# tlkvstepan/PracticalDeepStereo_NIPS2018

Measured on AMD Instinct MI355X. Metric: stereo pairs/sec, 960x540 D=192, Matching+Regularization+SubpixelMap hot path, higher is better.
Workload: dtype f32; 1 GPU; configs[1]: 960x540 pair padded to 576x960, D=192 (48 matching planes, 96 cost planes), batch 1, eval mode, random-init weights seed 0; parallelism=single GPU, launch=eager, whole pairs round-robin over 3 HIP streams

## Files before the change

practicaldeepstereo_nips2018_amd/csrc/conv2d_t8.hip:

```cpp
#include <atomic>
#include <type_traits>

#include "common.hpp"

namespace pds {

namespace {

constexpr int C2_THREADS = 256;
constexpr int C2_CIN = 64, C2_COUT = 8, C2_KC = 4, C2_CHUNKS = C2_CIN / C2_KC;
constexpr int C2_TY = 16, C2_NB = 2, C2_TX = 16 * C2_NB, C2_RP = C2_TY / 8;
constexpr int C2_YT = C2_TY + 2, C2_XT = C2_TX + 2, C2_RS = 36;
constexpr int C2_PART = C2_YT * C2_RS * 8;
constexpr int C2_BUF = 2 * C2_PART;
constexpr int C2_AFRAGS = C2_CHUNKS * 3 * 2;
constexpr int C2_ABYTES = C2_AFRAGS * 64 * 8;
constexpr int C2_NPOS = C2_YT * C2_XT;
constexpr int C2_POS = (C2_NPOS + C2_THREADS - 1) / C2_THREADS;
static_assert(C2_RS >= C2_XT, "LDS row");
typedef float f32x4 __attribute__((ext_vector_type(4)));
typedef _Float16 f16x4 __attribute__((ext_vector_type(4)));

struct C2Args {
    Src a, b;
    const float* __restrict__ w;
    const float* __restrict__ bias;
    float* __restrict__ out;
    int N, D, H, W;
    int lrelu;
    int tiles_x, tiles_y, tiles;
};

__device__ __forceinline__ void c2_split(const float (&v)[4], f16x4& hi, f16x4& lo) {
    pds_u32x2 h, l;
    split_quad_f16(v, h, l);
    hi = __builtin_bit_cast(f16x4, h);
    lo = __builtin_bit_cast(f16x4, l);
}

struct C2Scales {
    float ws, as, unscale;
};
__device__ __forceinline__ float c2_uniform(float v) {
    return __builtin_bit_cast(float, __builtin_amdgcn_readfirstlane(__builtin_bit_cast(int, v)));
}
__device__ __forceinline__ C2Scales c2_scales(const C2Args& A, bool two, float* red) {
    float m[3] = {0.f, 0.f, 0.f};
    for (int i = threadIdx.x; i < C2_COUT * C2_CIN * 9; i += blockDim.x) m[0] = fmaxf(m[0], fabsf(A.w[i]));
    for (int i = threadIdx.x; i < A.a.bound_n; i += blockDim.x) {
        const float v = fabsf(A.a.bound[i]);
        m[1] = fmaxf(m[1], v == v ? v : __builtin_inff());
    }
    if (two)
        for (int i = threadIdx.x; i < A.b.bound_n; i += blockDim.x) {
            const float v = fabsf(A.b.bound[i]);
            m[2] = fmaxf(m[2], v == v ? v : __builtin_inff());
        }
    const int wave = threadIdx.x >> 6, waves = (blockDim.x + 63) >> 6;
#pragma unroll
    for (int k = 0; k < 3; ++k) {
        m[k] = wave_max(m[k]);
        if ((threadIdx.x & 63) == 0) red[wave * 3 + k] = m[k];
    }
    __syncthreads();
    float r[3] = {0.f, 0.f, 0.f};
    for (int w = 0; w < waves; ++w)
#pragma unroll
        for (int k = 0; k < 3; ++k) r[k] = fmaxf(r[k], red[w * 3 + k]);
    __syncthreads();
    C2Scales S;
    S.ws = c2_uniform(pow2_scale(r[0], kHalfTarget));
    S.as = c2_uniform(pow2_scale(r[1] + r[2], kHalfTarget));
    S.unscale = c2_uniform((1.f / S.ws) * (1.f / S.as));
    return S;
}

}

template <bool TWO, bool NA, bool NB2>
__global__ __launch_bounds__(C2_THREADS, 2) void conv2d_t8_kernel(const C2Args A) {
    extern __shared__ __attribute__((aligned(16))) unsigned char lds[];
    unsigned char* abuf = lds;
    unsigned char* ibuf = lds + C2_ABYTES;

    const int tid = threadIdx.x;
    const int lane = tid & 63;
    const int wave = __builtin_amdgcn_readfirstlane(tid >> 6);
    const int n16 = lane & 15, q = lane >> 4;
    const size_t plane = (size_t)A.H * A.W;
    const size_t cstride = (size_t)A.D * plane;
    const int cbytes = (int)(cstride * sizeof(float));
    const __amdgpu_buffer_rsrc_t ra = __builtin_amdgcn_make_buffer_rsrc(
        const_cast<float*>(A.a.p), 0, (int)((size_t)A.N * C2_CIN * cstride * sizeof(float)), 0x00020000);
    const __amdgpu_buffer_rsrc_t rb = __builtin_amdgcn_make_buffer_rsrc(
        const_cast<float*>(TWO ? A.b.p : A.a.p), 0, (int)((size_t)A.N * C2_CIN * cstride * sizeof(float)), 0x00020000);
    const __amdgpu_buffer_rsrc_t ro = __builtin_amdgcn_make_buffer_rsrc(
        A.out, 0, (int)((size_t)A.N * C2_COUT * cstride * sizeof(float)), 0x00020000);

    const C2Scales SC = c2_scales(A, TWO, reinterpret_cast<float*>(ibuf));
    for (int e = tid; e < C2_CHUNKS * 3 * 64; e += C2_THREADS) {
        const int l = e & 63, f = e >> 6;
        const int m = l & 15, oc = m >> 1, py = m & 1, yi = l >> 4, dy = yi - py;
        const int chunk = f / 3, dx = f % 3;
        float wv[4];
#pragma unroll
        for (int i = 0; i < 4; ++i)
            wv[i] = (dy >= 0 && dy <= 2)
                        ? A.w[((size_t)oc * C2_CIN + chunk * C2_KC + i) * 9 + dy * 3 + dx] * SC.ws
                        : 0.f;
        f16x4 hi, lo;
        c2_split(wv, hi, lo);
        *reinterpret_cast<f16x4*>(abuf + ((size_t)(f * 2 + 0) * 64 + l) * 8) = hi;
        *reinterpret_cast<f16x4*>(abuf + ((size_t)(f * 2 + 1) * 64 + l) * 8) = lo;
    }

    const int xcd = blockIdx.x & 7, slot = blockIdx.x >> 3, per_xcd = gridDim.x >> 3;
    const int t_end = (int)(((long long)(xcd + 1) * A.tiles) >> 3);
    const int t_first = (int)(((long long)xcd * A.tiles) >> 3) + slot;
    const int my_tiles = t_first < t_end ? (t_end - t_first + per_xcd - 1) / per_xcd : 0;
    const int total_chunks = my_tiles * C2_CHUNKS;

    int lo_off[C2_POS];
#pragma unroll
    for (int k = 0; k < C2_POS; ++k) {
        const int p = min(tid + C2_THREADS * k, C2_NPOS - 1);
        lo_off[k] = ((p / C2_XT) * C2_RS + p % C2_XT) * 8;
    }

    struct TilePos {
        int nb, d, y0, x0;
    };
    auto tile_pos = [&](int local) {
        const int t = t_first + min(local, my_tiles - 1) * per_xcd;
        TilePos p;
        p.x0 = (t % A.tiles_x) * C2_TX;
        int r = t / A.tiles_x;
        p.y0 = (r % A.tiles_y) * C2_TY;
        r /= A.tiles_y;
        p.d = r % A.D;
        p.nb = r / A.D;
        return p;
    };

    unsigned goff[C2_POS], goff_n[C2_POS];
    float inside[C2_POS], inside_n[C2_POS];
    int sbase = 0, sbase_n = 0;
    int gidx = 0, gidx_n = 0, gch = 0, gch_n = 0;
    const int stride_a = (NA && A.a.per_plane) ? A.D : 1, stride_b = (TWO && NB2 && A.b.per_plane) ? A.D : 1;
    auto prepare = [&](int local, unsigned* off, float* in, int& sb, int& gi, int& gc) {
        const TilePos P = tile_pos(local);
#pragma unroll
        for (int k = 0; k < C2_POS; ++k) {
            const int p = min(tid + C2_THREADS * k, C2_NPOS - 1);
            const int y = P.y0 + p / C2_XT - 1, x = P.x0 + p % C2_XT - 1;
            const bool ok = (unsigned)y < (unsigned)A.H && (unsigned)x < (unsigned)A.W;
            in[k] = ok ? 1.f : 0.f;
            off[k] = ok ? (unsigned)((size_t)y * A.W + x) * 4u : ~0u;
        }
        sb = (int)(((size_t)P.nb * C2_CIN * A.D + P.d) * plane * sizeof(float));
        gi = (NA && A.a.per_plane) ? P.nb * C2_CIN * A.D + P.d : P.nb * C2_CIN;
        gc = (TWO && NB2 && A.b.per_plane) ? P.nb * C2_CIN * A.D + P.d : P.nb * C2_CIN;
    };

    constexpr int DEPTH = 4;
    float va[DEPTH][C2_POS][C2_KC], vb[DEPTH][C2_POS][C2_KC];
    float vs[DEPTH][C2_KC], vh[DEPTH][C2_KC], vs2[DEPTH][C2_KC], vh2[DEPTH][C2_KC];
    float inside_regs[DEPTH][C2_POS];
    auto fetch = [&](int g, auto set_c) {
        constexpr int SET = decltype(set_c)::value;
        const int c0 = (g % C2_CHUNKS) * C2_KC;
        const int soff = __builtin_amdgcn_readfirstlane(sbase + c0 * cbytes);
#pragma unroll
        for (int k = 0; k < C2_POS; ++k) {
#pragma unroll
            for (int ch = 0; ch < C2_KC; ++ch) {
                va[SET][k][ch] =
                    __builtin_bit_cast(float, __builtin_amdgcn_raw_buffer_load_b32(ra, goff[k], soff + ch * cbytes, 0));
                if (TWO)
                    vb[SET][k][ch] = __builtin_bit_cast(
                        float, __builtin_amdgcn_raw_buffer_load_b32(rb, goff[k], soff + ch * cbytes, 0));
            }
            inside_regs[SET][k] = inside[k];
        }
#pragma unroll
        for (int ch = 0; ch < C2_KC; ++ch) {
            if (NA) {
                const int gi = __builtin_amdgcn_readfirstlane(gidx + (c0 + ch) * stride_a);
                vs[SET][ch] = A.a.scale[gi];
                vh[SET][ch] = A.a.shift[gi];
            }
            if (TWO && NB2) {
                const int gi = __builtin_amdgcn_readfirstlane(gch + (c0 + ch) * stride_b);
                vs2[SET][ch] = A.b.scale[gi];
                vh2[SET][ch] = A.b.shift[gi];
            }
        }
    };
    auto stash = [&](unsigned char* buf, auto set_c) {
        constexpr int SET = decltype(set_c)::value;
        float cs[C2_KC], cs2[C2_KC], chs[C2_KC];
#pragma unroll
        for (int ch = 0; ch < C2_KC; ++ch) {
            cs[ch] = NA ? vs[SET][ch] * SC.as : SC.as;
            cs2[ch] = (TWO && NB2) ? vs2[SET][ch] * SC.as : SC.as;
            chs[ch] = ((NA ? vh[SET][ch] : 0.f) + ((TWO && NB2) ? vh2[SET][ch] : 0.f)) * SC.as;
        }
#pragma unroll
        for (int k = 0; k < C2_POS; ++k) {
            float v[4];
#pragma unroll
            for (int ch = 0; ch < C2_KC; ++ch) {
                float t = cs[ch] * va[SET][k][ch];
                if (TWO) t = fmaf(cs2[ch], vb[SET][k][ch], t);
                if (NA || (TWO && NB2)) t = fmaf(chs[ch], inside_regs[SET][k], t);
                v[ch] = t;
            }
            f16x4 hi, lo;
            c2_split(v, hi, lo);
            *reinterpret_cast<f16x4*>(buf + lo_off[k]) = hi;
            *reinterpret_cast<f16x4*>(buf + C2_PART + lo_off[k]) = lo;
        }
    };

    const float bscale = SC.ws * SC.as;
    const float bias0 = (A.bias ? A.bias[2 * q] : 0.f) * bscale, bias1 = (A.bias ? A.bias[2 * q + 1] : 0.f) * bscale;
    const int b_base = ((2 * C2_RP * wave + q) * C2_RS + n16) * 8;
    const unsigned out_lane = (unsigned)((size_t)(2 * q) * cstride + n16) * 4u;
    const unsigned out_c1 = (unsigned)cstride * 4u;

    using S0 = std::integral_constant<int, 0>;
    using S1 = std::integral_constant<int, 1>;
    using S2 = std::integral_constant<int, 2>;
    using S3 = std::integral_constant<int, 3>;
    int fetched_tile = -1;
    auto fetch_chunk = [&](int g, auto set_c) {
        const int gf = min(g, total_chunks - 1);
        if (gf / C2_CHUNKS != fetched_tile) {
            fetched_tile = gf / C2_CHUNKS;
            prepare(fetched_tile, goff, inside, sbase, gidx, gch);
        }
        fetch(gf, set_c);
    };
    if (total_chunks > 0) {
        fetch_chunk(0, S0());
        stash(ibuf, S0());
        fetch_chunk(1, S1());
        fetch_chunk(2, S2());
        fetch_chunk(3, S3());
    }
    __syncthreads();

    f32x4 acc[C2_RP][C2_NB];
    TilePos Pcur = tile_pos(0);
    auto step = [&](int g, auto set_stash, auto set_fetch) {
        const int c = g % C2_CHUNKS;
        if (c == 0) {
            Pcur = tile_pos(g / C2_CHUNKS);
#pragma unroll
            for (int p = 0; p < C2_RP; ++p)
#pragma unroll
                for (int j = 0; j < C2_NB; ++j) acc[p][j] = f32x4{bias0, bias0, bias1, bias1};
        }
        const int gf = min(g + DEPTH, total_chunks - 1);
        const bool new_tile = gf / C2_CHUNKS != fetched_tile;
        if (new_tile) prepare(gf / C2_CHUNKS, goff_n, inside_n, sbase_n, gidx_n, gch_n);
        fetched_tile = gf / C2_CHUNKS;

        const unsigned char* buf = ibuf + (g & 1) * C2_BUF + b_base;
        stash(ibuf + ((g + 1) & 1) * C2_BUF, set_stash);
#pragma unroll
        for (int k = 0; k < C2_POS; ++k) {
            inside[k] = new_tile ? inside_n[k] : inside[k];
            goff[k] = new_tile ? goff_n[k] : goff[k];
        }
        sbase = new_tile ? sbase_n : sbase;
        gidx = new_tile ? gidx_n : gidx;
        gch = new_tile ? gch_n : gch;
        fetch(gf, set_fetch);
        const unsigned char* af = abuf + ((size_t)c * 3 * 2 * 64 + lane) * 8;
#pragma unroll
        for (int dx = 0; dx < 3; ++dx) {
            const f16x4 a_hi = *reinterpret_cast<const f16x4*>(af + (dx * 2 + 0) * 512);
            const f16x4 a_lo = *reinterpret_cast<const f16x4*>(af + (dx * 2 + 1) * 512);
#pragma unroll
            for (int p = 0; p < C2_RP; ++p)
#pragma unroll
                for (int j = 0; j < C2_NB; ++j) {
                    const unsigned char* bp = buf + ((2 * p) * C2_RS + 16 * j + dx) * 8;
                    const f16x4 b_hi = *reinterpret_cast<const f16x4*>(bp);
                    const f16x4 b_lo = *reinterpret_cast<const f16x4*>(bp + C2_PART);
                    acc[p][j] = __builtin_amdgcn_mfma_f32_16x16x16f16(a_hi, b_lo, acc[p][j], 0, 0, 0);
                    acc[p][j] = __builtin_amdgcn_mfma_f32_16x16x16f16(a_lo, b_hi, acc[p][j], 0, 0, 0);
                    acc[p][j] = __builtin_amdgcn_mfma_f32_16x16x16f16(a_hi, b_hi, acc[p][j], 0, 0, 0);
                }
        }
#pragma unroll
        for (int i = 0; i < 3 * C2_RP * C2_NB * 3; ++i) {
            __builtin_amdgcn_sched_group_barrier(0x008, 1, 0);
            __builtin_amdgcn_sched_group_barrier(0x100, 1, 0);
            __builtin_amdgcn_sched_group_barrier(0x002, 4, 0);
            __builtin_amdgcn_sched_group_barrier(0x200, 1, 0);
            __builtin_amdgcn_sched_group_barrier(0x020, 1, 0);
        }
        if (c == C2_CHUNKS - 1) {
            const int out_base = (int)((size_t)Pcur.nb * C2_COUT * cstride * sizeof(float));
#pragma unroll
            for (int p = 0; p < C2_RP; ++p)
#pragma unroll
                for (int r = 0; r < 4; ++r) {
                    const int h = r >> 1, y = Pcur.y0 + 2 * (C2_RP * wave + p) + (r & 1);
                    const int row_bytes = __builtin_amdgcn_readfirstlane(
                        out_base + (int)(((size_t)Pcur.d * A.H + min(y, A.H - 1)) * A.W + Pcur.x0) * (int)sizeof(float));
#pragma unroll
                    for (int j = 0; j < C2_NB; ++j) {
                        float t = acc[p][j][r] * SC.unscale;
                        if (A.lrelu) t = fmaxf(t, t * kLeakySlope);
                        const bool ok = y < A.H && Pcur.x0 + 16 * j + n16 < A.W;
                        __builtin_amdgcn_raw_buffer_store_b32(__builtin_bit_cast(int, t), ro,
                                                              ok ? out_lane + (h ? out_c1 : 0u) + 64u * j : ~0u, row_bytes, 0);
                    }
                }
        }
        __syncthreads();
    };
    for (int g = 0; g < total_chunks; g += 4) {
        step(g, S1(), S0());
        step(g + 1, S2(), S1());
        step(g + 2, S3(), S2());
        step(g + 3, S0(), S3());
    }
}

constexpr int C2W_THREADS = 512;
constexpr int C2W_MAXW = 352;
typedef unsigned u32x4 __attribute__((ext_vector_type(4)));

template <bool TWO, int NBH, int C2W_TY, int C2W_ITEMS>
__global__ __launch_bounds__(C2W_THREADS, 2) void conv2d_t8w_kernel(const C2Args A) {
    constexpr int C2W_YT = C2W_TY + 2;
    extern __shared__ __attribute__((aligned(16))) unsigned char lds[];
    unsigned char* abuf = lds;
    unsigned char* ibuf = lds + C2_ABYTES;
    const int RSW = A.W + 4, QW = A.W >> 2;
    const int part_bytes = C2W_YT * RSW * 8, buf_bytes = 2 * part_bytes;

    const int tid = threadIdx.x;
    const int lane = tid & 63;
    const int wave = __builtin_amdgcn_readfirstlane(tid >> 6);
    const int pair = wave & 3, half = wave >> 2;
    const int n16 = lane & 15, q = lane >> 4;
    const size_t plane = (size_t)A.H * A.W;
    const size_t cstride = (size_t)A.D * plane;
    const int cbytes = (int)(cstride * sizeof(float));
    const __amdgpu_buffer_rsrc_t ra = __builtin_amdgcn_make_buffer_rsrc(
        const_cast<float*>(A.a.p), 0, (int)((size_t)A.N * C2_CIN * cstride * sizeof(float)), 0x00020000);
    const __amdgpu_buffer_rsrc_t rb = __builtin_amdgcn_make_buffer_rsrc(
        const_cast<float*>(TWO ? A.b.p : A.a.p), 0, (int)((size_t)A.N * C2_CIN * cstride * sizeof(float)), 0x00020000);
    const __amdgpu_buffer_rsrc_t ro = __builtin_amdgcn_make_buffer_rsrc(
        A.out, 0, (int)((size_t)A.N * C2_COUT * cstride * sizeof(float)), 0x00020000);

    const C2Scales SC = c2_scales(A, TWO, reinterpret_cast<float*>(ibuf));
    for (int e = tid; e < C2_CHUNKS * 3 * 64; e += C2W_THREADS) {
        const int l = e & 63, f = e >> 6;
        const int m = l & 15, oc = m >> 1, py = m & 1, yi = l >> 4, dy = yi - py;
        const int chunk = f / 3, dx = f % 3;
        float wv[4];
#pragma unroll
        for (int i = 0; i < 4; ++i)
            wv[i] = (dy >= 0 && dy <= 2)
                        ? A.w[((size_t)oc * C2_CIN + chunk * C2_KC + i) * 9 + dy * 3 + dx] * SC.ws
                        : 0.f;
        f16x4 hi, lo;
        c2_split(wv, hi, lo);
        *reinterpret_cast<f16x4*>(abuf + ((size_t)(f * 2 + 0) * 64 + l) * 8) = hi;
        *reinterpret_cast<f16x4*>(abuf + ((size_t)(f * 2 + 1) * 64 + l) * 8) = lo;
    }
    for (int e = tid; e < 2 * 2 * C2W_YT * 2; e += C2W_THREADS) {
        const int side = e & 1, row = e >> 1;
        *reinterpret_cast<unsigned long long*>(ibuf + ((size_t)row * RSW + (side ? A.W + 2 : 1)) * 8) = 0ull;
    }

    const int xcd = blockIdx.x & 7, slot = blockIdx.x >> 3, per_xcd = gridDim.x >> 3;
    const int t_end = (int)(((long long)(xcd + 1) * A.tiles) >> 3);
    const int t_first = (int)(((long long)xcd * A.tiles) >> 3) + slot;
    const int my_tiles = t_first < t_end ? (t_end - t_first + per_xcd - 1) / per_xcd : 0;
    const int total_chunks = my_tiles * C2_CHUNKS;

    int item_row[C2W_ITEMS], item_col[C2W_ITEMS], lo_off[C2W_ITEMS], lo_step[C2W_ITEMS];
    bool item_ok[C2W_ITEMS];
#pragma unroll
    for (int k = 0; k < C2W_ITEMS; ++k) {
        item_ok[k] = tid + C2W_THREADS * k < C2W_YT * QW;
        const int it = min(tid + C2W_THREADS * k, C2W_YT * QW - 1);
        item_row[k] = it / QW;
        item_col[k] = 4 * (it % QW);
        lo_off[k] = item_ok[k] ? (item_row[k] * RSW + 2 + item_col[k]) * 8 : 0;
        lo_step[k] = item_ok[k] ? 16 : 0;
    }

    struct TilePos {
        int nb, d, y0;
    };
    auto tile_pos = [&](int local) {
        const int t = t_first + min(local, my_tiles - 1) * per_xcd;
        TilePos p;
        p.y0 = (t % A.tiles_y) * C2W_TY;
        const int r = t / A.tiles_y;
        p.d = r % A.D;
        p.nb = r / A.D;
        return p;
    };

    unsigned goff[C2W_ITEMS], goff_n[C2W_ITEMS];
    float inside[C2W_ITEMS], inside_n[C2W_ITEMS];
    int sbase = 0, sbase_n = 0;
    int gidx = 0, gidx_n = 0;
    const int stride_a = A.a.per_plane ? A.D : 1;
    auto prepare = [&](int local, unsigned* off, float* in, int& sb, int& gi) {
        const TilePos P = tile_pos(local);
#pragma unroll
        for (int k = 0; k < C2W_ITEMS; ++k) {
            const int y = P.y0 + item_row[k] - 1;
            const bool ok = (unsigned)y < (unsigned)A.H && item_ok[k];
            in[k] = ok ? 1.f : 0.f;
            off[k] = ok ? (unsigned)((size_t)y * A.W + item_col[k]) * 4u : ~0u;
        }
        sb = (int)(((size_t)P.nb * C2_CIN * A.D + P.d) * plane * sizeof(float));
        gi = A.a.per_plane ? P.nb * C2_CIN * A.D + P.d : P.nb * C2_CIN;
    };

    f32x4 va[2][C2W_ITEMS][C2_KC], vb[2][C2W_ITEMS][C2_KC];
    float vs[2][C2_KC], vh[2][C2_KC];
    float inside_regs[2][C2W_ITEMS];
    auto fetch = [&](int g, auto set_c) {
        constexpr int SET = decltype(set_c)::value;
        const int c0 = (g % C2_CHUNKS) * C2_KC;
        const int soff = __builtin_amdgcn_readfirstlane(sbase + c0 * cbytes);
#pragma unroll
        for (int k = 0; k < C2W_ITEMS; ++k) {
#pragma unroll
            for (int ch = 0; ch < C2_KC; ++ch) {
                va[SET][k][ch] = __builtin_bit_cast(
                    f32x4, __builtin_amdgcn_raw_buffer_load_b128(ra, goff[k], soff + ch * cbytes, 0));
                if (TWO)
                    vb[SET][k][ch] = __builtin_bit_cast(
                        f32x4, __builtin_amdgcn_raw_buffer_load_b128(rb, goff[k], soff + ch * cbytes, 0));
            }
            inside_regs[SET][k] = inside[k];
        }
#pragma unroll
        for (int ch = 0; ch < C2_KC; ++ch) {
            const int gi = __builtin_amdgcn_readfirstlane(gidx + (c0 + ch) * stride_a);
            vs[SET][ch] = A.a.scale[gi];
            vh[SET][ch] = A.a.shift[gi];
        }
    };
    typedef _Float16 f16x8 __attribute__((ext_vector_type(8)));
    auto stash = [&](unsigned char* buf, auto set_c) {
        constexpr int SET = decltype(set_c)::value;
        float cs[C2_KC], chs[C2_KC];
#pragma unroll
        for (int ch = 0; ch < C2_KC; ++ch) {
            cs[ch] = vs[SET][ch] * SC.as;
            chs[ch] = vh[SET][ch] * SC.as;
        }
#pragma unroll
        for (int k = 0; k < C2W_ITEMS; ++k)
#pragma unroll
            for (int pp = 0; pp < 2; ++pp) {
                f16x8 hi2, lo2;
#pragma unroll
                for (int e = 0; e < 2; ++e) {
                    const int px = 2 * pp + e;
                    float v[4];
#pragma unroll
                    for (int ch = 0; ch < C2_KC; ++ch) {
                        float t = cs[ch] * va[SET][k][ch][px];
                        if (TWO) t = fmaf(SC.as, vb[SET][k][ch][px], t);
                        v[ch] = fmaf(chs[ch], inside_regs[SET][k], t);
                    }
                    f16x4 hi, lo;
                    c2_split(v, hi, lo);
#pragma unroll
                    for (int i = 0; i < 4; ++i) {
                        hi2[4 * e + i] = hi[i];
                        lo2[4 * e + i] = lo[i];
                    }
                }
                *reinterpret_cast<f16x8*>(buf + lo_off[k] + pp * lo_step[k]) = hi2;
                *reinterpret_cast<f16x8*>(buf + part_bytes + lo_off[k] + pp * lo_step[k]) = lo2;
            }
    };

    const float bscale = SC.ws * SC.as;
    const float bias0 = (A.bias ? A.bias[2 * q] : 0.f) * bscale, bias1 = (A.bias ? A.bias[2 * q + 1] : 0.f) * bscale;
    const int b_base = ((2 * pair + q) * RSW + 16 * half * NBH + n16 + 1) * 8;
    const unsigned out_lane = (unsigned)((size_t)(2 * q) * cstride + 16 * half * NBH + n16) * 4u;
    const unsigned out_c1 = (unsigned)cstride * 4u;

    using S0 = std::integral_constant<int, 0>;
    using S1 = std::integral_constant<int, 1>;
    int fetched_tile = -1;
    auto fetch_chunk = [&](int g, auto set_c) {
        const int gf = min(g, total_chunks - 1);
        if (gf / C2_CHUNKS != fetched_tile) {
            fetched_tile = gf / C2_CHUNKS;
            prepare(fetched_tile, goff, inside, sbase, gidx);
        }
        fetch(gf, set_c);
    };
    __syncthreads();
    if (total_chunks > 0) {
        fetch_chunk(0, S0());
        stash(ibuf, S0());
        fetch_chunk(1, S1());
        fetch_chunk(2, S0());
    }
    __syncthreads();

    f32x4 acc[NBH];
    TilePos Pcur = tile_pos(0);
#ifdef PDS_C2W_TIMING
    long long tmw[5] = {0, 0, 0, 0, 0};
#endif
    auto step = [&](int g, auto set_c) {
        const int c = g % C2_CHUNKS;
        if (c == 0) {
            Pcur = tile_pos(g / C2_CHUNKS);
#pragma unroll
            for (int j = 0; j < NBH; ++j) acc[j] = f32x4{bias0, bias0, bias1, bias1};
        }
        const int gf = min(g + 3, total_chunks - 1);
        const bool new_tile = gf / C2_CHUNKS != fetched_tile;
        if (new_tile) prepare(gf / C2_CHUNKS, goff_n, inside_n, sbase_n, gidx_n);
        fetched_tile = gf / C2_CHUNKS;

        const unsigned char* buf = ibuf + (g & 1) * buf_bytes + b_base;
#ifdef PDS_C2W_TIMING
        const long long tt0 = __builtin_readcyclecounter();
#endif
        stash(ibuf + ((g + 1) & 1) * buf_bytes, set_c);
#ifdef PDS_C2W_TIMING
        asm volatile("s_waitcnt lgkmcnt(0)" ::: "memory");
        const long long tt1 = __builtin_readcyclecounter();
#endif
#pragma unroll
        for (int k = 0; k < C2W_ITEMS; ++k) {
            inside[k] = new_tile ? inside_n[k] : inside[k];
            goff[k] = new_tile ? goff_n[k] : goff[k];
        }
        sbase = new_tile ? sbase_n : sbase;
        gidx = new_tile ? gidx_n : gidx;
        fetch(gf, set_c);
#ifdef PDS_C2W_TIMING
        const long long tt2 = __builtin_readcyclecounter();
#endif
        const unsigned char* af = abuf + ((size_t)c * 3 * 2 * 64 + lane) * 8;
#pragma unroll
        for (int dx = 0; dx < 3; ++dx) {
            const f16x4 a_hi = *reinterpret_cast<const f16x4*>(af + (dx * 2 + 0) * 512);
            const f16x4 a_lo = *reinterpret_cast<const f16x4*>(af + (dx * 2 + 1) * 512);
#pragma unroll
            for (int j = 0; j < NBH; ++j) {
                const unsigned char* bp = buf + (16 * j + dx) * 8;
                const f16x4 b_hi = *reinterpret_cast<const f16x4*>(bp);
                const f16x4 b_lo = *reinterpret_cast<const f16x4*>(bp + part_bytes);
                acc[j] = __builtin_amdgcn_mfma_f32_16x16x16f16(a_hi, b_lo, acc[j], 0, 0, 0);
                acc[j] = __builtin_amdgcn_mfma_f32_16x16x16f16(a_lo, b_hi, acc[j], 0, 0, 0);
                acc[j] = __builtin_amdgcn_mfma_f32_16x16x16f16(a_hi, b_hi, acc[j], 0, 0, 0);
            }
        }
#ifndef PDS_C2W_TIMING
#pragma unroll
        for (int i = 0; i < 3 * NBH * 3; ++i) {
            __builtin_amdgcn_sched_group_barrier(0x008, 1, 0);
            __builtin_amdgcn_sched_group_barrier(0x100, 1, 0);
            __builtin_amdgcn_sched_group_barrier(0x002, 4, 0);
            __builtin_amdgcn_sched_group_barrier(0x200, 1, 0);
            __builtin_amdgcn_sched_group_barrier(0x020, 1, 0);
        }
#else
        const long long tt3 = __builtin_readcyclecounter();
        tmw[0] += tt1 - tt0; tmw[1] += tt2 - tt1; tmw[2] += tt3 - tt2;
#endif
        if (c == C2_CHUNKS - 1) {
            const int out_base = (int)((size_t)Pcur.nb * C2_COUT * cstride * sizeof(float));
#pragma unroll
            for (int r = 0; r < 4; ++r) {
                const int h = r >> 1, y = Pcur.y0 + 2 * pair + (r & 1);
                const int row_bytes = __builtin_amdgcn_readfirstlane(
                    out_base + (int)(((size_t)Pcur.d * A.H + min(y, A.H - 1)) * A.W) * (int)sizeof(float));
#pragma unroll
                for (int j = 0; j < NBH; ++j) {
                    float t = acc[j][r] * SC.unscale;
                    if (A.lrelu) t = fmaxf(t, t * kLeakySlope);
                    const bool ok = 2 * pair < C2W_TY && y < A.H && 16 * (half * NBH + j) + n16 < A.W;
                    __builtin_amdgcn_raw_buffer_store_b32(__builtin_bit_cast(int, t), ro,
                                                          ok ? out_lane + (h ? out_c1 : 0u) + 64u * j : ~0u, row_bytes, 0);
                }
            }
        }
#ifdef PDS_C2W_TIMING
        const long long tt4 = __builtin_readcyclecounter();
#endif
        __syncthreads();
#ifdef PDS_C2W_TIMING
        tmw[3] += __builtin_readcyclecounter() - tt4;
        tmw[4] += 1;
#endif
    };
#ifdef PDS_C2W_TIMING
    const long long t_all = __builtin_readcyclecounter();
#endif
    for (int g = 0; g < total_chunks; g += 2) {
        step(g, S1());
        step(g + 1, S0());
    }
#ifdef PDS_C2W_TIMING
    if (lane == 0 && (blockIdx.x % 61) == 0 && (wave == 0 || wave == 5))
        printf("[t8w] wg %d wave %d: total %lld | stash(+wait) %lld fetch-issue %lld mfma %lld barrier %lld over %lld chunks (%d tiles)\n",
               (int)blockIdx.x, wave, (long long)__builtin_readcyclecounter() - t_all, tmw[0], tmw[1], tmw[2], tmw[3], tmw[4], my_tiles);
#endif
}

namespace {

bool c2t8_enabled() {
    static const bool on = []() {
        const char* e = debug_switch("PDS_CONV2D_T8");
        return !(e && e[0] == '0');
    }();
    return on;
}

template <bool TWO, bool NA, bool NB2>
int launch_c2t8(const C2Args& A, hipStream_t s) {
    constexpr size_t lds_bytes = (size_t)C2_ABYTES + 2 * C2_BUF;
    static std::atomic<unsigned> attr_done{0};
    if (DeviceOnce once{attr_done}) {
        (void)hipFuncSetAttribute(reinterpret_cast<const void*>(&conv2d_t8_kernel<TWO, NA, NB2>),
                                  hipFuncAttributeMaxDynamicSharedMemorySize, (int)(160 * 1024));
    }
    int wgs = 512;
    if (wgs > A.tiles) wgs = (A.tiles + 7) / 8 * 8;
    hipLaunchKernelGGL((conv2d_t8_kernel<TWO, NA, NB2>), dim3(wgs), dim3(C2_THREADS), lds_bytes, s, A);
    return check_launch("conv2d_t8");
}

}

bool c2t8_wide(const ConvLayer& L) {
    static const bool on = []() {
        const char* e = debug_switch("PDS_CONV2D_T8W");
        return !(e && e[0] == '0');
    }();
    if (!on) return false;
    if (!L.a.scale || (L.b.p && L.b.scale)) return false;
    return (L.in.w & 3) == 0 && L.in.w >= 64 && L.in.w <= C2W_MAXW && L.in.h >= 8;
}

template <bool TWO, int NBH, int TY, int ITEMS>
int launch_c2t8w(C2Args& A, hipStream_t s) {
    A.tiles_x = 1;
    A.tiles_y = (A.H + TY - 1) / TY;
    A.tiles = A.N * A.D * A.tiles_y;
    const size_t lds_bytes = (size_t)C2_ABYTES + 2 * 2 * (size_t)(TY + 2) * (A.W + 4) * 8 + 2 * (size_t)(A.W + 4) * 8 + 256;
    static std::atomic<unsigned> attr_done{0};
    static int cus[32] = {0};
    int dev = 0;
    (void)hipGetDevice(&dev);
    if (DeviceOnce once{attr_done}) {
        (void)hipFuncSetAttribute(reinterpret_cast<const void*>(&conv2d_t8w_kernel<TWO, NBH, TY, ITEMS>),
                                  hipFuncAttributeMaxDynamicSharedMemorySize, (int)(160 * 1024));
        int n = 0;
        (void)hipDeviceGetAttribute(&n, hipDeviceAttributeMultiprocessorCount, dev);
        cus[dev & 31] = n > 0 ? n : 256;
    }
    int wgs = cus[dev & 31] / 8 * 8;
    if (wgs > A.tiles) wgs = (A.tiles + 7) / 8 * 8;
    const int probe = probe_before("conv2d_t8w", s);
    hipLaunchKernelGGL((conv2d_t8w_kernel<TWO, NBH, TY, ITEMS>), dim3(wgs), dim3(C2W_THREADS), lds_bytes, s, A);
    probe_after(probe, A.tiles, s);
    return check_launch("conv2d_t8w");
}

int c2t8w_rows(int w) {
    static const int forced = []() {
        const char* e = debug_switch("PDS_CONV2D_T8W_ROWS");
        return e ? atoi(e) : 0;
    }();
    if (forced == 8 || forced == 6) return forced;
    return 8 * (w >> 2) <= C2W_THREADS ? 6 : 8;
}

bool conv2d_t8_supported(const ConvLayer& L) {
    if (!c2t8_enabled()) return false;
    if (L.kd != 1 || L.stride != 1 || L.in.c != C2_CIN || L.out_g.c != C2_COUT) return false;
    if (L.l0A || L.side_out || L.plane_weight_sets > 0) return false;
    if (!L.a.bounded) return false;
    if (L.b.p && !L.b.bounded) return false;
    if (L.b.p && L.b.bcast_d) return false;
    if ((size_t)L.in.n * C2_CIN * L.in.d * L.in.h * L.in.w >= ((size_t)1 << 29)) return false;
    const long tiles = (long)L.in.n * L.in.d * ((L.in.h + C2_TY - 1) / C2_TY) * ((L.in.w + C2_TX - 1) / C2_TX);
    return tiles < (1L << 30);
}

int launch_conv2d_t8(const ConvLayer& L, hipStream_t s) {
    C2Args A;
    A.a = L.a;
    A.b = L.b;
    A.w = L.weight;
    A.bias = L.bias;
    A.out = L.out;
    A.N = L.in.n;
    A.D = L.in.d;
    A.H = L.in.h;
    A.W = L.in.w;
    A.lrelu = L.lrelu;
    A.tiles_x = (A.W + C2_TX - 1) / C2_TX;
    A.tiles_y = (A.H + C2_TY - 1) / C2_TY;
    A.tiles = A.N * A.D * A.tiles_y * A.tiles_x;
    if (!A.a.bound || A.a.bound_n <= 0 || (L.b.p && (!A.b.bound || A.b.bound_n <= 0)))
        return set_error(-1, "conv2d_t8: a source without a range bound");
    if (c2t8_wide(L)) {
        const int blocks = (A.W + 15) / 16, nbh = (blocks + 1) / 2;
        const int rows = c2t8w_rows(A.W), items = ((rows + 2) * (A.W >> 2) + C2W_THREADS - 1) / C2W_THREADS;
        if (nbh <= 8 && rows == 6 && items == 1)
            return L.b.p ? launch_c2t8w<true, 8, 6, 1>(A, s) : launch_c2t8w<false, 8, 6, 1>(A, s);
        if (nbh <= 8) return L.b.p ? launch_c2t8w<true, 8, 8, 2>(A, s) : launch_c2t8w<false, 8, 8, 2>(A, s);
        return L.b.p ? launch_c2t8w<true, 11, 8, 2>(A, s) : launch_c2t8w<false, 11, 8, 2>(A, s);
    }
    const bool na = L.a.scale != nullptr, nb2 = L.b.p && L.b.scale;
    if (L.b.p) {
        if (na) return nb2 ? launch_c2t8<true, true, true>(A, s) : launch_c2t8<true, true, false>(A, s);
        return nb2 ? launch_c2t8<true, false, true>(A, s) : launch_c2t8<true, false, false>(A, s);
    }
    return na ? launch_c2t8<false, true, false>(A, s) : launch_c2t8<false, false, false>(A, s);
}

}
```

Baseline: 431.6 pairs/s.

## Add warp-specialized wide conv2d kernel with dedicated staging and MFMA waves

Adds a new wide-tile conv2d kernel in which four waves only issue MFMAs while another 256 threads act as staging waves. The staging waves prefetch inputs through a deep register ring of buffer loads, apply normalization, and write split f16 hi/lo data into double-buffered LDS. Each MFMA wave covers a full row width (NB=16 or 22 blocks). The kernel is on by default and selected ahead of the existing t8w path. It aims to overlap global fetch with MFMA compute without the old kernel's interleaved stash and fetch phases, at the cost of higher register pressure and half the waves doing no math.

```diff
diff --git a/practicaldeepstereo_nips2018_amd/csrc/conv2d_t8.hip b/practicaldeepstereo_nips2018_amd/csrc/conv2d_t8.hip
--- a/practicaldeepstereo_nips2018_amd/csrc/conv2d_t8.hip
+++ b/practicaldeepstereo_nips2018_amd/csrc/conv2d_t8.hip
@@ -621,6 +621,294 @@
         printf("[t8w] wg %d wave %d: total %lld | stash(+wait) %lld fetch-issue %lld mfma %lld barrier %lld over %lld chunks (%d tiles)\n",
                (int)blockIdx.x, wave, (long long)__builtin_readcyclecounter() - t_all, tmw[0], tmw[1], tmw[2], tmw[3], tmw[4], my_tiles);
 #endif
+}
+
+namespace {
+
+constexpr int C2R_STAGERS = 256;
+typedef const __attribute__((address_space(4))) float c2r_cfloat;
+
+__device__ __forceinline__ void c2r_barrier() { asm volatile("s_waitcnt lgkmcnt(0)\n\ts_barrier" ::: "memory"); }
+
+struct C2rList {
+    int t_first, per_xcd, my_tiles, total_chunks;
+};
+__device__ __forceinline__ C2rList c2r_list(const C2Args& A) {
+    C2rList L;
+    const int xcd = blockIdx.x & 7, slot = blockIdx.x >> 3;
+    L.per_xcd = gridDim.x >> 3;
+    const int t_end = (int)(((long long)(xcd + 1) * A.tiles) >> 3);
+    L.t_first = (int)(((long long)xcd * A.tiles) >> 3) + slot;
+    L.my_tiles = L.t_first < t_end ? (t_end - L.t_first + L.per_xcd - 1) / L.per_xcd : 0;
+    L.total_chunks = L.my_tiles * C2_CHUNKS;
+    return L;
+}
+template <int TY>
+__device__ __forceinline__ void c2r_tile(const C2Args& A, const C2rList& L, int local, int& nb, int& d, int& y0) {
+    const int t = L.t_first + local * L.per_xcd;
+    y0 = (t % A.tiles_y) * TY;
+    const int r = t / A.tiles_y;
+    d = r % A.D;
+    nb = r / A.D;
+}
+
+template <int NB, int TY>
+__device__ __forceinline__ void c2r_mfma_waves(const C2Args& A, const C2Scales& SC, const C2rList& L,
+                                               const unsigned char* lds, int wave, int lane) {
+    const unsigned char* abuf = lds;
+    const unsigned char* ibuf = lds + C2_ABYTES;
+    const int RSW = A.W + 4;
+    const int part_bytes = (TY + 2) * RSW * 8, buf_bytes = 2 * part_bytes;
+    const int n16 = lane & 15, q = lane >> 4;
+    const size_t cstride = (size_t)A.D * A.H * A.W;
+    const __amdgpu_buffer_rsrc_t ro = __builtin_amdgcn_make_buffer_rsrc(
+        A.out, 0, (int)((size_t)A.N * C2_COUT * cstride * sizeof(float)), 0x00020000);
+    const float bscale = SC.ws * SC.as;
+    const float bias0 = (A.bias ? A.bias[2 * q] : 0.f) * bscale, bias1 = (A.bias ? A.bias[2 * q + 1] : 0.f) * bscale;
+    const int b_base = ((2 * wave + q) * RSW + n16 + 1) * 8;
+    const unsigned out_lane = (unsigned)((size_t)(2 * q) * cstride + n16) * 4u;
+    const unsigned out_c1 = (unsigned)cstride * 4u;
+    const bool active = 2 * wave < TY;
+    __builtin_amdgcn_s_setprio(3);
+
+    c2r_barrier();
+    for (int t = 0; t < L.my_tiles; ++t) {
+        f32x4 acc[NB];
+#pragma unroll
+        for (int j = 0; j < NB; ++j) acc[j] = f32x4{bias0, bias0, bias1, bias1};
+        for (int c = 0; c < C2_CHUNKS; ++c) {
+            if (active) {
+                const unsigned char* buf = ibuf + (c & 1) * buf_bytes + b_base;
+                const unsigned char* af = abuf + ((size_t)c * 3 * 2 * 64 + lane) * 8;
+#pragma unroll
+                for (int dx = 0; dx < 3; ++dx) {
+                    const f16x4 a_hi = *reinterpret_cast<const f16x4*>(af + (dx * 2 + 0) * 512);
+                    const f16x4 a_lo = *reinterpret_cast<const f16x4*>(af + (dx * 2 + 1) * 512);
+#pragma unroll
+                    for (int j = 0; j < NB; ++j) {
+                        const unsigned char* bp = buf + (16 * j + dx) * 8;
+                        const f16x4 b_hi = *reinterpret_cast<const f16x4*>(bp);
+                        const f16x4 b_lo = *reinterpret_cast<const f16x4*>(bp + part_bytes);
+                        acc[j] = __builtin_amdgcn_mfma_f32_16x16x16f16(a_hi, b_lo, acc[j], 0, 0, 0);
+                        acc[j] = __builtin_amdgcn_mfma_f32_16x16x16f16(a_lo, b_hi, acc[j], 0, 0, 0);
+                        acc[j] = __builtin_amdgcn_mfma_f32_16x16x16f16(a_hi, b_hi, acc[j], 0, 0, 0);
+                    }
+                }
+            }
+            c2r_barrier();
+        }
+        if (active) {
+            int nb, d, y0;
+            c2r_tile<TY>(A, L, t, nb, d, y0);
+            const int out_base = (int)((size_t)nb * C2_COUT * cstride * sizeof(float));
+#pragma unroll
+            for (int r = 0; r < 4; ++r) {
+                const int h = r >> 1, y = y0 + 2 * wave + (r & 1);
+                const int row_bytes = __builtin_amdgcn_readfirstlane(
+                    out_base + (int)(((size_t)d * A.H + min(y, A.H - 1)) * A.W) * (int)sizeof(float));
+#pragma unroll
+                for (int j = 0; j < NB; ++j) {
+                    float v = acc[j][r] * SC.unscale;
+                    if (A.lrelu) v = fmaxf(v, v * kLeakySlope);
+                    const bool ok = y < A.H && 16 * j + n16 < A.W;
+                    __builtin_amdgcn_raw_buffer_store_b32(__builtin_bit_cast(int, v), ro,
+                                                          ok ? out_lane + (h ? out_c1 : 0u) + 64u * j : ~0u, row_bytes, 0);
+                }
+            }
+        }
+    }
+}
+
+template <bool TWO, int TY, int P, int DEPTH>
+__device__ __forceinline__ void c2r_staging_waves(const C2Args& A, const C2Scales& SC, const C2rList& L,
+                                                  unsigned char* lds, int sid) {
+    constexpr int YT = TY + 2;
+    constexpr int U = (P == 1 || P == 2 || P == 4) ? DEPTH / P : DEPTH;
+    static_assert(DEPTH == 4 && (U == 1 || U == 2 || U == 4), "register ring");
+    unsigned char* ibuf = lds + C2_ABYTES;
+    const int RSW = A.W + 4, QW = A.W >> 2;
+    const int part_bytes = YT * RSW * 8, buf_bytes = 2 * part_bytes;
+    const size_t plane = (size_t)A.H * A.W;
+    const size_t cstride = (size_t)A.D * plane;
+    const int cbytes = (int)(cstride * sizeof(float));
+    const __amdgpu_buffer_rsrc_t ra = __builtin_amdgcn_make_buffer_rsrc(
+        const_cast<float*>(A.a.p), 0, (int)((size_t)A.N * C2_CIN * cstride * sizeof(float)), 0x00020000);
+    const __amdgpu_buffer_rsrc_t rb = __builtin_amdgcn_make_buffer_rsrc(
+        const_cast<float*>(TWO ? A.b.p : A.a.p), 0, (int)((size_t)A.N * C2_CIN * cstride * sizeof(float)), 0x00020000);
+    const int total = L.total_chunks;
+
+    int item_row[P], item_col[P], lo_off[P], lo_step[P];
+    bool item_ok[P];
+#pragma unroll
+    for (int k = 0; k < P; ++k) {
+        item_ok[k] = sid + C2R_STAGERS * k < YT * QW;
+        const int it = min(sid + C2R_STAGERS * k, YT * QW - 1);
+        item_row[k] = it / QW;
+        item_col[k] = 4 * (it % QW);
+        lo_off[k] = item_ok[k] ? (item_row[k] * RSW + 2 + item_col[k]) * 8 : 0;
+        lo_step[k] = item_ok[k] ? 16 : 0;
+    }
+
+    unsigned goff[P];
+    float inside[P];
+    int sbase = 0, gidx = 0, fetched_tile = -1;
+    const int stride_a = A.a.per_plane ? A.D : 1;
+    auto prepare = [&](int local) {
+        int nb, d, y0;
+        c2r_tile<TY>(A, L, local, nb, d, y0);
+#pragma unroll
+        for (int k = 0; k < P; ++k) {
+            const int y = y0 + item_row[k] - 1;
+            const bool ok = (unsigned)y < (unsigned)A.H && item_ok[k];
+            inside[k] = ok ? 1.f : 0.f;
+            goff[k] = ok ? (unsigned)((size_t)y * A.W + item_col[k]) * 4u : ~0u;
+        }
+        sbase = (int)(((size_t)nb * C2_CIN * A.D + d) * plane * sizeof(float));
+        gidx = A.a.per_plane ? nb * C2_CIN * A.D + d : nb * C2_CIN;
+    };
+
+    f32x4 va[DEPTH][C2_KC], vb[DEPTH][C2_KC];
+    float vs[DEPTH][C2_KC], vh[DEPTH][C2_KC];
+    float inside_regs[DEPTH];
+    auto fetch = [&](int g, int k, int set) {
+        const bool live = g < total;
+        const int gc = live ? g : total - 1;
+        if (gc / C2_CHUNKS != fetched_tile) {
+            fetched_tile = gc / C2_CHUNKS;
+            prepare(fetched_tile);
+        }
+        const int c0 = (gc % C2_CHUNKS) * C2_KC;
+        const int soff = __builtin_amdgcn_readfirstlane(sbase + c0 * cbytes);
+        const unsigned off = live ? goff[k] : ~0u;
+#pragma unroll
+        for (int ch = 0; ch < C2_KC; ++ch) {
+            va[set][ch] = __builtin_bit_cast(f32x4, __builtin_amdgcn_raw_buffer_load_b128(ra, off, soff + ch * cbytes, 0));
+            if (TWO)
+                vb[set][ch] =
+                    __builtin_bit_cast(f32x4, __builtin_amdgcn_raw_buffer_load_b128(rb, off, soff + ch * cbytes, 0));
+        }
+        inside_regs[set] = inside[k];
+        const c2r_cfloat* sc = (const c2r_cfloat*)A.a.scale;
+        const c2r_cfloat* sh = (const c2r_cfloat*)A.a.shift;
+#pragma unroll
+        for (int ch = 0; ch < C2_KC; ++ch) {
+            const int gi = __builtin_amdgcn_readfirstlane(gidx + (c0 + ch) * stride_a);
+            vs[set][ch] = sc[gi];
+            vh[set][ch] = sh[gi];
+        }
+    };
+    typedef _Float16 f16x8 __attribute__((ext_vector_type(8)));
+    auto stash = [&](unsigned char* buf, int k, int set) {
+        constexpr int LPU = TWO ? 2 * C2_KC : C2_KC;
+        if (TWO)
+            asm volatile("s_waitcnt vmcnt(%8)"
+                         : "+v"(va[set][0]), "+v"(va[set][1]), "+v"(va[set][2]), "+v"(va[set][3]), "+v"(vb[set][0]),
+                           "+v"(vb[set][1]), "+v"(vb[set][2]), "+v"(vb[set][3])
+                         : "n"((DEPTH - 1) * LPU)
+                         : "memory");
+        else
+            asm volatile("s_waitcnt vmcnt(%4)"
+                         : "+v"(va[set][0]), "+v"(va[set][1]), "+v"(va[set][2]), "+v"(va[set][3])
+                         : "n"((DEPTH - 1) * LPU)
+                         : "memory");
+        float cs[C2_KC], chs[C2_KC];
+#pragma unroll
+        for (int ch = 0; ch < C2_KC; ++ch) {
+            cs[ch] = vs[set][ch] * SC.as;
+            chs[ch] = vh[set][ch] * SC.as;
+        }
+#pragma unroll
+        for (int pp = 0; pp < 2; ++pp) {
+            f16x8 hi2, lo2;
+#pragma unroll
+            for (int e = 0; e < 2; ++e) {
+                const int px = 2 * pp + e;
+                float v[4];
+#pragma unroll
+                for (int ch = 0; ch < C2_KC; ++ch) {
+                    float t = cs[ch] * va[set][ch][px];
+                    if (TWO) t = fmaf(SC.as, vb[set][ch][px], t);
+                    v[ch] = fmaf(chs[ch], inside_regs[set], t);
+                }
+                f16x4 hi, lo;
+                c2_split(v, hi, lo);
+#pragma unroll
+                for (int i = 0; i < 4; ++i) {
+                    hi2[4 * e + i] = hi[i];
+                    lo2[4 * e + i] = lo[i];
+                }
+            }
+            *reinterpret_cast<f16x8*>(buf + lo_off[k] + pp * lo_step[k]) = hi2;
+            *reinterpret_cast<f16x8*>(buf + part_bytes + lo_off[k] + pp * lo_step[k]) = lo2;
+        }
+    };
+    auto stage = [&](int gn, auto i_c) {
+        constexpr int I = decltype(i_c)::value;
+        unsigned char* buf = ibuf + (gn & 1) * buf_bytes;
+#pragma unroll
+        for (int k = 0; k < P; ++k) {
+            const int set = ((I + 1) * P + k) % DEPTH;
+            stash(buf, k, set);
+            fetch(gn + (k + DEPTH) / P, (k + DEPTH) % P, set);
+        }
+    };
+
+    if (total > 0) {
+#pragma unroll
+        for (int u = 0; u < DEPTH; ++u) fetch(u / P, u % P, u);
+        stage(0, std::integral_constant<int, U - 1>());
+    }
+    c2r_barrier();
+    static_assert(C2_CHUNKS % U == 0, "steps per tile");
+    auto step = [&](int g, auto i_c) {
+        stage(g + 1, i_c);
+        c2r_barrier();
+    };
+    for (int g = 0; g < total; g += U) {
+        step(g, std::integral_constant<int, 0>());
+        if constexpr (U > 1) step(g + 1, std::integral_constant<int, 1>());
+        if constexpr (U > 2) {
+            step(g + 2, std::integral_constant<int, 2>());
+            step(g + 3, std::integral_constant<int, 3>());
+        }
+    }
+}
+
+}
+
+template <bool TWO, int NB, int TY, int P>
+__global__ __launch_bounds__(C2W_THREADS, 1) void conv2d_t8w_rs_kernel(const C2Args A) {
+    extern __shared__ __attribute__((aligned(16))) unsigned char lds[];
+    unsigned char* abuf = lds;
+    unsigned char* ibuf = lds + C2_ABYTES;
+    const int tid = threadIdx.x;
+    const int wave = __builtin_amdgcn_readfirstlane(tid >> 6);
+    const int RSW = A.W + 4;
+
+    const C2Scales SC = c2_scales(A, TWO, reinterpret_cast<float*>(ibuf));
+    for (int e = tid; e < C2_CHUNKS * 3 * 64; e += C2W_THREADS) {
+        const int l = e & 63, f = e >> 6;
+        const int m = l & 15, oc = m >> 1, py = m & 1, yi = l >> 4, dy = yi - py;
+        const int chunk = f / 3, dx = f % 3;
+        float wv[4];
+#pragma unroll
+        for (int i = 0; i < 4; ++i)
+            wv[i] = (dy >= 0 && dy <= 2)
+                        ? A.w[((size_t)oc * C2_CIN + chunk * C2_KC + i) * 9 + dy * 3 + dx] * SC.ws
+                        : 0.f;
+        f16x4 hi, lo;
+        c2_split(wv, hi, lo);
+        *reinterpret_cast<f16x4*>(abuf + ((size_t)(f * 2 + 0) * 64 + l) * 8) = hi;
+        *reinterpret_cast<f16x4*>(abuf + ((size_t)(f * 2 + 1) * 64 + l) * 8) = lo;
+    }
+    for (int e = tid; e < 2 * 2 * (TY + 2) * 2; e += C2W_THREADS) {
+        const int side = e & 1, row = e >> 1;
+        *reinterpret_cast<unsigned long long*>(ibuf + ((size_t)row * RSW + (side ? A.W + 2 : 1)) * 8) = 0ull;
+    }
+    const C2rList L = c2r_list(A);
+    __syncthreads();
+    if (wave < 4) c2r_mfma_waves<NB, TY>(A, SC, L, lds, wave, tid & 63);
+    else c2r_staging_waves<TWO, TY, P, 4>(A, SC, L, lds, tid - C2R_STAGERS);
 }
 
 namespace {
@@ -680,6 +968,40 @@
     if (wgs > A.tiles) wgs = (A.tiles + 7) / 8 * 8;
     const int probe = probe_before("conv2d_t8w", s);
     hipLaunchKernelGGL((conv2d_t8w_kernel<TWO, NBH, TY, ITEMS>), dim3(wgs), dim3(C2W_THREADS), lds_bytes, s, A);
+    probe_after(probe, A.tiles, s);
+    return check_launch("conv2d_t8w");
+}
+
+bool c2t8w_rs() {
+    static const bool on = []() {
+        const char* e = debug_switch("PDS_CONV2D_T8W_RS");
+        return !(e && e[0] == '0');
+    }();
+    return on;
+}
+
+template <bool TWO, int NB, int TY, int P>
+int launch_c2t8w_rs(C2Args& A, hipStream_t s) {
+    A.tiles_x = 1;
+    A.tiles_y = (A.H + TY - 1) / TY;
+    A.tiles = A.N * A.D * A.tiles_y;
+    const size_t lds_bytes =
+        (size_t)C2_ABYTES + 2 * 2 * (size_t)(TY + 2) * (A.W + 4) * 8 + (size_t)max(0, 16 * NB - A.W) * 8;
+    static std::atomic<unsigned> attr_done{0};
+    static int cus[32] = {0};
+    int dev = 0;
+    (void)hipGetDevice(&dev);
+    if (DeviceOnce once{attr_done}) {
+        (void)hipFuncSetAttribute(reinterpret_cast<const void*>(&conv2d_t8w_rs_kernel<TWO, NB, TY, P>),
+                                  hipFuncAttributeMaxDynamicSharedMemorySize, (int)(160 * 1024));
+        int n = 0;
+        (void)hipDeviceGetAttribute(&n, hipDeviceAttributeMultiprocessorCount, dev);
+        cus[dev & 31] = n > 0 ? n : 256;
+    }
+    int wgs = cus[dev & 31] / 8 * 8;
+    if (wgs > A.tiles) wgs = (A.tiles + 7) / 8 * 8;
+    const int probe = probe_before("conv2d_t8w", s);
+    hipLaunchKernelGGL((conv2d_t8w_rs_kernel<TWO, NB, TY, P>), dim3(wgs), dim3(C2W_THREADS), lds_bytes, s, A);
     probe_after(probe, A.tiles, s);
     return check_launch("conv2d_t8w");
 }
@@ -725,6 +1047,12 @@
     if (c2t8_wide(L)) {
         const int blocks = (A.W + 15) / 16, nbh = (blocks + 1) / 2;
         const int rows = c2t8w_rows(A.W), items = ((rows + 2) * (A.W >> 2) + C2W_THREADS - 1) / C2W_THREADS;
+        if (c2t8w_rs()) {
+            if (nbh <= 8 && rows == 6 && items == 1)
+                return L.b.p ? launch_c2t8w_rs<true, 16, 6, 2>(A, s) : launch_c2t8w_rs<false, 16, 6, 2>(A, s);
+            if (nbh <= 8) return L.b.p ? launch_c2t8w_rs<true, 16, 8, 3>(A, s) : launch_c2t8w_rs<false, 16, 8, 3>(A, s);
+            return L.b.p ? launch_c2t8w_rs<true, 22, 8, 4>(A, s) : launch_c2t8w_rs<false, 22, 8, 4>(A, s);
+        }
         if (nbh <= 8 && rows == 6 && items == 1)
             return L.b.p ? launch_c2t8w<true, 8, 6, 1>(A, s) : launch_c2t8w<false, 8, 6, 1>(A, s);
         if (nbh <= 8) return L.b.p ? launch_c2t8w<true, 8, 8, 2>(A, s) : launch_c2t8w<false, 8, 8, 2>(A, s);
```

After: 432.3 pairs/s (median of 6 runs). About the same (+0.2%).
